# p3achyjr/p3achygo

Hardware: AMD Instinct MI355X
Metric: self-play positions/sec at 1/8 MI355X, b12c256btl3 19x19 n=32 (higher is better)
Workload: dtype f16; 1 GPU; b12c256btl3 random-init, self-play: C++ host (Gumbel MCTS n=32, default k<=5, selected k=5) -> p3hip_run over batches of 1024 leaf positions -> results back to the search; one step = one round = one engine batch of each of the 8 game groups = 8192 positions; batch_per_gpu=1024, concurrent_games_per_gpu=8192, game_groups_per_gpu=8, lanes_per_group=1, ladder_node_budget=0, parallelism=games sharded x1, no collective

## Files before the change

p3achygo_amd/csrc/conv_any.hip:

```cpp
#include "conv_any.h"

#include <hip/hip_runtime.h>

#include <atomic>
#include <cstdlib>

#include "conv_core.h"

namespace p3 {

namespace {

struct InitAnyArgs { InitArgs a; int C; };
struct Conv1x1AnyArgs { Conv1x1Args a; int cin, cout; };
struct LConvAnyArgs { LConvArgs a; int nip, ncp; };
struct BDenseAnyArgs { BDenseArgs a; int C; };

struct FeatOff {
  static constexpr int color = 4, komi = 8, board = 12, last = 376, atari = 416, two = 777,
                       three = 1138, ladder = 1499, size = 1860;
};

}

// ... 23 lines not shown
        return (_Float16)((signed char)f[off + loc] == color ? 1.0f : 0.0f);
      };
      auto opp = [&](int off) {
        return (_Float16)((signed char)f[off + loc] == -color ? 1.0f : 0.0f);
      };
      lo[0] = our(FeatOff::board); lo[1] = opp(FeatOff::board);
      lo[7] = our(FeatOff::atari); hi[0] = opp(FeatOff::atari);
      hi[1] = our(FeatOff::two); hi[2] = opp(FeatOff::two);
      hi[3] = our(FeatOff::three); hi[4] = opp(FeatOff::three);
      hi[5] = our(FeatOff::ladder); hi[6] = opp(FeatOff::ladder);
      const int y = (loc * 3450) >> 16, xx = loc - y * kBL;
#pragma unroll
      for (int m = 0; m < 5; ++m) {
        const int* lm = (const int*)(f + FeatOff::last + m * 8);
        if (lm[0] == y && lm[1] == xx) lo[2 + m] = (_Float16)1.0f;
      }
      const int s = G::PADTOP + y * G::S + xx;
      *(h8*)(smem + s * G::SLOTB) = lo;
      *(h8*)(smem + s * G::SLOTB + 16) = hi;
    }
    float gsv[8];
    gsv[0] = color == 1 ? 1.0f : 0.0f;
    gsv[1] = color == 1 ? 0.0f : 1.0f;
#pragma unroll
    for (int m = 0; m < 5; ++m) {
      const int* lm = (const int*)(f + FeatOff::last + m * 8);
      gsv[2 + m] = (lm[0] == 19 && lm[1] == 0) ? 1.0f : 0.0f;
    }
    gsv[7] = (color == 1 ? -1.0f : 1.0f) * (*(const float*)(f + FeatOff::komi)) / 15.0f;

    static_assert(kConvAnyMaxC <= kWG, "one thread per channel");
    float* bias_lds = (float*)(smem + kRingOff + ring_bytes(CP));
    const int tc = launder((int)threadIdx.x);
    if (tc < C) {
      float b = a.game_b[tc];
#pragma unroll
      for (int k = 0; k < 8; ++k) b += a.game_w[k * C + tc] * gsv[k];
      bias_lds[tc] = b;
    }

#pragma unroll 1
    for (int cp = 0; cp < C / CP; ++cp) {
      f32x16 acc[2][T::NT];
      acc_zero<G, CP>(acc);
      conv_segment<G, CP, 5, 28>(ring, smem, acc);
#pragma unroll
      for (int mt = 0; mt < 2; ++mt)
#pragma unroll
        for (int g4 = 0; g4 < 4; ++g4) {
          const int c = cp * CP + acc_chan<G, CP>(mt, g4);
          const f32x4 bias = *(const f32x4*)(bias_lds + c);
#pragma unroll
          for (int j = 0; j < T::NT; ++j) {
            const int t = lg + j * T::LG;
            if (t >= G::NT_TOTAL) continue;
            const int r = t * 32 + lr;
            int loc;
            if (!row_valid<G::S>(r, loc)) continue;
            h4 o;
#pragma unroll
            for (int i = 0; i < 4; ++i) o[i] = (_Float16)(acc[mt][j][g4 * 4 + i] + bias[i]);
            *(h4*)(a.x + ((size_t)pos * (C / 8) + (c >> 3)) * (kNLoc * 8) + loc * 8 + h * 4) = o;
          }
        }
    }
    lds_barrier();
  }
  ring_drain();
}

template <int CB, int CP, bool PRE, int EPI>
__global__ void __launch_bounds__(kWG, 2) k_conv1x1_any(Conv1x1AnyArgs aa) {
// ... 395 lines not shown
```

p3achygo_amd/csrc/conv_core.h:

```cpp
#pragma once
#include <hip/hip_runtime.h>
#include <stdint.h>

namespace p3 {

typedef _Float16 h8 __attribute__((ext_vector_type(8)));
typedef _Float16 h4 __attribute__((ext_vector_type(4)));
typedef _Float16 h2 __attribute__((ext_vector_type(2)));
typedef float f32x16 __attribute__((ext_vector_type(16)));
typedef float f32x4 __attribute__((ext_vector_type(4)));

constexpr int kWG = 512;
constexpr int kNLoc = 361;
constexpr int kBL = 19;
constexpr int kKMS = 4;
constexpr int kRingSlots = 3;
constexpr int kRingDepth = 2;
#ifndef P3_RING_DEPTH4
#define P3_RING_DEPTH4 2
#endif
constexpr int kRingDepth4 = P3_RING_DEPTH4;
constexpr int ring_slot_bytes(int cout_pass, int kms = kKMS) { return kms * cout_pass * 32; }
constexpr int ring_bytes(int cout_pass, int kms = kKMS, int depth = kRingDepth) { return (depth + 1) * ring_slot_bytes(cout_pass, kms); }

// ... 201 lines not shown

template <class G>
__device__ __forceinline__ int tile_slot0(int t) {
  int p = t / G::NT_POS;
  int tt = t - p * G::NT_POS;
  return p * G::PSLOTS + G::PADTOP + tt * 32;
}

template <int OFF>
__device__ __forceinline__ h8 lds_read128(uint32_t addr) {
  h8 r;
  asm volatile("ds_read_b128 %0, %1 offset:%2" : "=v"(r) : "v"(addr), "i"(OFF));
  return r;
}
template <int N>
__device__ __forceinline__ void wait_lgkm() {
  asm volatile("s_waitcnt lgkmcnt(%0)" ::"n"(N));
  __builtin_amdgcn_sched_barrier(0);
}

__device__ __forceinline__ void wait_lgkm_n(int n) {
  switch (n) {
    case 0: wait_lgkm<0>(); break;
    case 1: wait_lgkm<1>(); break;
    case 2: wait_lgkm<2>(); break;
    case 3: wait_lgkm<3>(); break;
    case 4: wait_lgkm<4>(); break;
    case 5: wait_lgkm<5>(); break;
    case 6: wait_lgkm<6>(); break;
    default: wait_lgkm<7>(); break;
  }
}

template <class G, int COUT_PASS, int KW, int NTAPS_PAD, bool SWAP = false, int NTn = 0>
__device__ __forceinline__ void conv_segment(Ring<ring_slot_bytes(COUT_PASS, G::KMS), G::NW, G::RD>& ring, char* smem,
                                             f32x16 (&acc)[2][NTn]) {
  using T = Tiling<G, COUT_PASS>;
  static_assert(NTn == T::NT, "accumulator shape");
  constexpr int NQ = G::CB / 16;
  constexpr int NK16 = NTAPS_PAD * NQ;
  constexpr int U = (NK16 <= 28) ? NK16 : 3 * NQ;
  constexpr int NOUT = NK16 / U;
  constexpr int NLD = 2 + T::NT;
  static_assert(NK16 % U == 0 && U % T::KMS == 0 && (NOUT == 1 || (U % 3 == 0 && U % NQ == 0)) &&
                NK16 >= 3, "segment shape");
  const int lane = threadIdx.x & 63;
  const int wid = __builtin_amdgcn_readfirstlane(threadIdx.x >> 6);
  const int cg = wid % T::CG, lg = wid / T::CG;
  const int lr = lane & 31, h = lane >> 5;

  int slot0[T::NT];
#pragma unroll
  for (int j = 0; j < T::NT; ++j) {
    int t = lg + j * T::LG;
    if (t >= G::NT_TOTAL) t = lg;
    slot0[j] = tile_slot0<G>(t) + lr;
  }
  const uint32_t a_off = (uint32_t)((h * COUT_PASS + cg * 64 + lr) * 16);
  uint32_t a_addr = 0;
  uint32_t b_base[T::NT];
  h8 fa[3][2], fb[3][T::NT];

  auto fetch_piece = [&](int o, int v, int pc) {
    const int vv = v % U;
    const int ob = o + v / U;
    const int q = vv % NQ;
    const int buf = v % 3;
    constexpr int KB = COUT_PASS * 32;
    const int kk = vv % T::KMS;
    if (pc == 0) {
      if (kk == 0) a_addr = ring_acquire(ring, smem) + a_off;
      if (vv % NQ == 0) {
        const int tap = ob * (U / NQ) + vv / NQ;
        int shift = 0;
        if (KW > 1) {
          const int ky = tap / KW, kx = tap - ky * KW;
          shift = (tap < KW * KW) ? (ky - KW / 2) * G::S + (kx - KW / 2) : 0;
        }
#pragma unroll
// ... 21 lines not shown
        case 6: fb[buf][j] = lds_read128<192>(b_base[j]); break;
        case 7: fb[buf][j] = lds_read128<224>(b_base[j]); break;
        case 8: fb[buf][j] = lds_read128<256>(b_base[j]); break;
        case 9: fb[buf][j] = lds_read128<288>(b_base[j]); break;
        case 10: fb[buf][j] = lds_read128<320>(b_base[j]); break;
        case 11: fb[buf][j] = lds_read128<352>(b_base[j]); break;
        case 12: fb[buf][j] = lds_read128<384>(b_base[j]); break;
        case 13: fb[buf][j] = lds_read128<416>(b_base[j]); break;
        case 14: fb[buf][j] = lds_read128<448>(b_base[j]); break;
        case 15: fb[buf][j] = lds_read128<480>(b_base[j]); break;
        case 16: fb[buf][j] = lds_read128<512>(b_base[j]); break;
        case 17: fb[buf][j] = lds_read128<544>(b_base[j]); break;
        case 18: fb[buf][j] = lds_read128<576>(b_base[j]); break;
        case 19: fb[buf][j] = lds_read128<608>(b_base[j]); break;
        case 20: fb[buf][j] = lds_read128<640>(b_base[j]); break;
        case 21: fb[buf][j] = lds_read128<672>(b_base[j]); break;
        case 22: fb[buf][j] = lds_read128<704>(b_base[j]); break;
        default: fb[buf][j] = lds_read128<736>(b_base[j]); break;
      }
    }
  };
  auto fetch = [&](int o, int v) {
#pragma unroll
    for (int pc = 0; pc < 1 + T::NT; ++pc) fetch_piece(o, v, pc);
  };

  fetch(0, 0);
  fetch(0, 1);
#pragma unroll 1
  for (int o = 0; o < NOUT; ++o) {
#pragma unroll
    for (int u = 0; u < U; ++u) {
      const bool last_body = (NOUT == 1) || (o + 1 == NOUT);
      if (u + 1 < U || !last_body) wait_lgkm<NLD>();
      else wait_lgkm<0>();
      const bool do_fetch = (u + 2 < U) || !last_body;
#pragma unroll
      for (int m = 0; m < 2 * T::NT; ++m) {
        const int mt = m / T::NT, j = m % T::NT;
        acc[mt][j] = SWAP ? __builtin_amdgcn_mfma_f32_32x32x16_f16(fb[u % 3][j], fa[u % 3][mt], acc[mt][j], 0, 0, 0)
                          : __builtin_amdgcn_mfma_f32_32x32x16_f16(fa[u % 3][mt], fb[u % 3][j], acc[mt][j], 0, 0, 0);
        if (m < 1 + T::NT) {
          __builtin_amdgcn_sched_barrier(0);
          if (do_fetch) fetch_piece(o, u + 2, m);
          __builtin_amdgcn_sched_barrier(0);
        }
      }
    }
  }
}

template <class G, int COUT_PASS, int NTn>
__device__ __forceinline__ void acc_zero(f32x16 (&acc)[2][NTn]) {
#pragma unroll
  for (int mt = 0; mt < 2; ++mt)
#pragma unroll
    for (int j = 0; j < NTn; ++j)
#pragma unroll
      for (int i = 0; i < 16; ++i) acc[mt][j][i] = 0.0f;
}

template <class G, int COUT_PASS>
__device__ __forceinline__ int cg_of() {
  const int wid = __builtin_amdgcn_readfirstlane(threadIdx.x >> 6);
  return wid % Tiling<G, COUT_PASS>::CG;
}

template <class G, int COUT_PASS>
__device__ __forceinline__ int acc_chan(int mt, int g4) {
// ... 256 lines not shown
                                               const ResRegs<G, COUT_PASS, NTn>& rr,
                                               _Float16* __restrict__ x) {
#pragma unroll
  for (int j = 0; j < NTn; ++j)
#pragma unroll
    for (int kp = 0; kp < 4; ++kp) {
      const int k0 = 2 * kp, k1 = 2 * kp + 1;
      h4 r0 = {0, 0, 0, 0}, r1 = {0, 0, 0, 0};
      if (RESIDUAL) residual_unpack<G, COUT_PASS, NTn>(rr, j, kp, r0, r1);
      h4 o0, o1;
#pragma unroll
      for (int i = 0; i < 4; ++i) {
        float v0 = acc[k0 >> 2][j][(k0 & 3) * 4 + i], v1 = acc[k1 >> 2][j][(k1 & 3) * 4 + i];
        if (RESIDUAL) { v0 += (float)r0[i]; v1 += (float)r1[i]; }
        o0[i] = (_Float16)v0;
        o1[i] = (_Float16)v1;
      }
      half_swap32(o0, o1);
      const h8 piece = {o0[0], o0[1], o0[2], o0[3], o1[0], o1[1], o1[2], o1[3]};
      if (rr.ok[j]) *(h8*)((char*)x + sgpr_offset(rr.pos_base * 2 + (size_t)kp * (2 * kNLoc * 8 * 2)) + (uint32_t)(rr.base[j] * 2u)) = piece;
    }
}

template <class G, int COUT_PASS, bool RESIDUAL, int NTn>
__device__ __forceinline__ void epilogue_to_global(f32x16 (&acc)[2][NTn],
                                                   _Float16* __restrict__ x, int C, int pos0,
                                                   int npos, int cofs) {
  ResRegs<G, COUT_PASS, NTn> rr;
  residual_addr<G, COUT_PASS, NTn>(rr, C, pos0, npos, cofs);
  if (RESIDUAL) residual_load<G, COUT_PASS, NTn>(rr, x);
  epilogue_store<G, COUT_PASS, RESIDUAL, NTn>(acc, rr, x);
}

}
```

p3achygo_amd/csrc/engine.cpp:

```cpp
#include <hip/hip_runtime.h>
#include <chrono>

#include <algorithm>
#include <atomic>
#include <cmath>
#include <cstdio>
#include <cstdlib>
#include <cstring>
#include <functional>
#include <map>
#include <memory>
#include <unordered_set>
#include <string>
#include <vector>

#include "../../include/p3hip.h"
#include "kernels.h"
#include "block_i8.h"
#include "conv_any.h"
#include "lconv_i8.h"
#include "slot_state.h"
#include "symmetry.h"
#include "transformer.h"

// ... 462 lines not shown
                   (C == 384 || p3::heads_fusable(C, wf.V));
  const bool arch_ok = (fused && bottleneck_ok) || layerwise || tfm ||
                       (i8f && fused_shape);
  if (!arch_ok || wf.H != 32 || !v_ok) {
    e->err = "unsupported architecture for the HIP engine (need a conv trunk (" P3HIP_CONV_SET "), or a transformer "
             "trunk (" P3HIP_TRANSFORMER_SET "); H=32, V in {32,48,64,80} (transformer: V in {32,48,64}, and 80 at "
             "d > 256))";
    return false;
  }
  if (any && e->int8) {
    e->err = std::string(e->i8f ? "INT8_FUSED" : "INT8") + " is not available for this conv trunk: P3HIP_FLAG_INT8 "
             "serves C = 384 / C_b = 192 btl or nbt blocks and C = 192 classic blocks, P3HIP_FLAG_INT8_FUSED serves "
             "C = 256 / C_b = 128 btl blocks with 1, 2 or 3 inner layers; the other widths run in fp16 only";
    return false;
  }
  e->conv_any = any || (e->conv_any_env && lw_shape && !e->int8);
  e->tfm = tfm;
  if (tfm) {
    e->tfm_heads = Cb;
    e->tfm_D = wf.model_C / Cb;
  }
  if (i8f && !i8f_ok) {
    e->err = "INT8_FUSED is available only for C = 256 / C_b = 128 trunks of btl blocks with 1, 2 or 3 inner layers "
             "(b12c256btl3 and its kin, broadcast blocks at any interval), and not together with P3HIP_FLAG_INT8; nbt and "
             "C = 128 trunks, the layer-wise trunks (P3HIP_FLAG_INT8 serves those) and the transformer are not served";
    return false;
  }
  if (e->int8 && !layerwise) {
    e->err = "INT8 is available only for layer-wise trunks (C = 384 / C_b = 192 btl or nbt blocks, C = 192 classic "
             "blocks); this trunk runs fused block kernels or the transformer";
    return false;
  }
  const int CB = layerwise ? p3::conv_any_slice(C) : (tfm ? 128 : Cb);
  const int CPI = layerwise ? p3::conv_any_init_pass(C) : 128;
  {
    std::vector<_Float16> s;
    const Tensor& w = wf.get("init_conv.w", (size_t)25 * 15 * C);
    for (int cp = 0; cp < C / CPI; ++cp)
      pack_segment(s, w.data, 25, 28, 15, C, 0, 16, cp * CPI, CPI);
    e->init_stream_off = add_stream(ar, s, e->init_nms, CPI);
    e->game_w_off = ar.add(wf.get("init_game.w", (size_t)8 * C).data, 8 * C * 4);
    e->game_b_off = ar.add(wf.get("init_game.b", (size_t)C).data, C * 4);
  }
  {
    static const bool want_blockw = getenv("P3HIP_BLOCKW") != nullptr && atoi(getenv("P3HIP_BLOCKW")) != 0;
    e->blockw = want_blockw && !i8f && C == 256 && Cb == 128 && wf.btype == 0 && wf.inner >= 1 && wf.inner <= 3;
    if (e->blockw) e->bcast_fuse = false;
  }
  bool have_xa = false;
  std::vector<std::pair<size_t, std::vector<_Float16>>> run_streams;
  std::vector<_Float16> head_stream, tail_stream;
  int head_of = -1, tail_of = -1;
  std::vector<std::function<void()>> layout;
  auto flush_run = [&]() {
    if (!run_streams.empty()) {
      auto rs_all = std::make_shared<std::vector<std::pair<size_t, std::vector<_Float16>>>>(std::move(run_streams));
      auto hs = std::make_shared<std::vector<_Float16>>(std::move(head_stream));
      auto ts = std::make_shared<std::vector<_Float16>>(std::move(tail_stream));
      const int h_of = head_of, t_of = tail_of;
      layout.push_back([&ar, e, rs_all, hs, ts, h_of, t_of, Cb]() {
        int nms_unused = 0;
        if (h_of >= 0) {
          add_stream(ar, *hs, nms_unused, Cb);
          BlockPlan& b = e->blocks[rs_all->front().first];
          b.head_of = h_of;
          b.head_bytes = hs->size() * 2;
          e->blocks[h_of].last_fused = true;
// ... 477 lines not shown
  a.prm = e->d_arena + run.prm_off;
  a.npos = npos;
  a.nblk = run.nblk;
  a.nwg = npos < e->n_cu ? npos : e->n_cu;
  a.stamps = e->d_bw_stamps;
  size_t size = sizeof a;
  void* cfg[] = {HIP_LAUNCH_PARAM_BUFFER_POINTER, &a, HIP_LAUNCH_PARAM_BUFFER_SIZE, &size, HIP_LAUNCH_PARAM_END};
  return e->check(hipModuleLaunchKernel(e->bw_fn, a.nwg, 1, 1, 256, 1, 1, 0, e->stream, nullptr, cfg), "launch k_blockw");
}

template <class Launch>
bool timed_launch(p3hip_engine* e, int* timed, Launch&& launch) {
  const bool on = timed && 2 * *timed + 1 < (int)e->blk_ev.size();
  if (on) hipEventRecord(e->blk_ev[2 * *timed], e->stream);
  if (!launch()) return false;
  if (on) hipEventRecord(e->blk_ev[2 * (*timed)++ + 1], e->stream);
  return true;
}

bool enqueue_forward(p3hip_engine* e, const Pass& p) {
  const WeightFile& wf = e->wf;
  const int C = wf.C, npos = p.npos;
  hipStream_t s = e->stream;
  const bool any = e->conv_any;
  auto conv1x1 = [&](int which, const p3::Conv1x1Args& a) {
    return any ? p3::launch_conv1x1_any(C, which, a, e->n_cu, s) : p3::launch_conv1x1(C, which, a, e->n_cu, s);
  };
  {
    p3::InitArgs a{};
    a.feats = p.feats; a.x = e->d_x; a.npos = npos;
    a.wstream = e->d_arena + e->init_stream_off; a.nms_total = e->init_nms;
    a.game_w = e->dev<float>(e->game_w_off); a.game_b = e->dev<float>(e->game_b_off);
    if (!e->check(e->conv_any ? p3::launch_init_any(C, a, grid_for(e, npos, 1), s)
                              : p3::launch_init(C, a, grid_for(e, npos, 1), s), "launch k_init")) return false;
  }
#ifdef P3_DIAG
  e->launch_index = 0;
#endif
  const int stop_block = e->stop_block;
  e->last_npos = npos;
  for (size_t bi = 0; bi < e->blocks.size(); ++bi) {
    if (stop_block >= 0 && (int)bi >= stop_block) return true;
    const BlockPlan& bp = e->blocks[bi];
    if (bp.kind == 5) {
      const int d = wf.model_C;
      const size_t per = (size_t)e->rows * p3::kTfmLPad * d;
      _Float16 *q = e->d_qkv, *k = q + per, *v = k + per, *o = e->d_t;
      p3::TfmQkvArgs a{e->d_x, q, k, v, npos, e->dev<float>(bp.tfm.rms_in), e->d_arena + bp.tfm.wqkv,
                       e->dev<float>(e->rope_cos_off), e->dev<float>(e->rope_sin_off)};
      if (!e->check(p3::launch_tfm_qkv(d, e->tfm_D, a, s), "launch k_tfm_qkv")) return false;
      const p3::TfmAttnArgs b{q, k, v, o, npos, e->tfm_heads};
      if (!timed_launch(e, p.timed, [&] { return e->check(p3::launch_tfm_attn(e->tfm_D, b, s), "launch k_tfm_attn"); }))
        return false;
      const p3::TfmFfnArgs f{o, e->d_x, npos, e->d_arena + bp.tfm.wo, e->dev<float>(bp.tfm.rms_out),
                             e->d_arena + bp.tfm.wgu, e->d_arena + bp.tfm.wdown};
      if (!e->check(p3::launch_tfm_ffn(d, f, s), "launch k_tfm_ffn")) return false;
    } else if (bp.kind == 3) {
      p3::Conv1x1Args c0{};
      c0.in = e->d_x; c0.out16 = e->d_t; c0.npos = npos;
      c0.wstream = e->d_arena + bp.stream_off; c0.nms_total = bp.nms;
      c0.scale = e->dev<float>(bp.bn[0].scale_off); c0.shift = e->dev<float>(bp.bn[0].shift_off);
      if (!bp.first_fused && !e->check(conv1x1(0, c0), "launch conv_first")) return false;
      p3::BDenseArgs d{};
      d.t = e->d_t; d.u = e->d_u; d.npos = npos;
      d.wstream = e->d_arena + bp.stream2_off; d.nms_total = bp.nms2;
      d.bias = e->dev<float>(bp.dense_bias_off);
      d.scale = e->dev<float>(bp.bn[1].scale_off); d.shift = e->dev<float>(bp.bn[1].shift_off);
// ... 790 lines not shown
```

p3achygo_amd/csrc/kernels.h:

```cpp
#pragma once
#include <hip/hip_runtime.h>
#include <stdint.h>

namespace p3 {

constexpr int kOffMoveLogits = 0;
constexpr int kOffMoveProbs = 362;
constexpr int kOffValueProbs = 724;
constexpr int kOffScoreProbs = 726;
constexpr int kOffOptProbs = 1526;
constexpr int kOffErr2 = 1888;
constexpr int kResultFloats = 1889;
constexpr int kOffOptLogits = 1889;
constexpr int kOffOutcomeLogits = 2251;
constexpr int kOffScoreLogits = 2253;
constexpr int kOffOwnership = 3053;
constexpr int kOffGamma = 3414;
constexpr int kOutStride = 3416;

constexpr int kMaxBlockLayers = 8;

constexpr int kMaxFuse = 6;
constexpr int kMaxRuns = 4, kMaxLaunchBlocks = 12;
struct BlockParams {
// ... 79 lines not shown
  const float* shift;
};

constexpr int heads_image_floats(int H, int V) {
  return 2 * H * H + 2 * H * V + 2 * H * V + (2 * H + 1) * V + V * 14 + V + V + 4 * H + 2 * H + 2 * H + H + H + H + H + H + V + V + V + 16;
}

struct HeadsArgs {
  const float* hp;
  const _Float16* x;
  const void* conv_a;
  const float* image;
  float* out;
  float* res;
  int npos;
  int V;
  const float *gbn_scale, *gbn_shift;
  const float *gd_w, *gd_b;
  const float *moves_w;
  const float *pass_w, *pass_b;
  const float *opt_moves_w;
  const float *opt_pass_w, *opt_pass_b;
  const float *oq_embed_w, *oq_embed_b;
  const float *oq_out_w, *oq_out_b;
  const float *own_w;
  const float *gamma_pre_w, *gamma_pre_b;
  const float *gamma_out_w, *gamma_out_b;
  const float *score_pre_w, *score_pre_b;
  const float *score_out_w, *score_out_b;
};

hipError_t launch_block(int C, int kind, int L, bool wg8, const BlockArgs& a, int n_cu, hipStream_t s);
int block_macro_step_bytes(int C, bool wg8);
hipError_t launch_init(int C, const InitArgs& a, int grid, hipStream_t s);
hipError_t launch_conv1x1(int C, int which, const Conv1x1Args& a, int n_cu, hipStream_t s);
hipError_t launch_bdense(int C, const BDenseArgs& a, int grid, hipStream_t s);
hipError_t launch_lconv(int kw, int cin, int cout, const LConvArgs& a, int n_cu, hipStream_t s);
hipError_t launch_heads(const HeadsArgs& a, int grid, hipStream_t s);
bool heads_fusable(int C, int V);
hipError_t launch_headsx(int C, const HeadsArgs& a, int n_cu, hipStream_t s);

constexpr int kCacheWays = 8;
struct CacheKey { unsigned long long lo, hi, sym; };
struct CacheArgs {
  const CacheKey* keys;
  int n;
  unsigned long long* tkeys;
  unsigned* tmeta;
  float* tvals;
  unsigned mask;
  unsigned run;
  int* hit;
  int* victim;
  const int* rows;
  const int* src;
  const int* idx;
  int m;
  int out_row0;
  float* out;
  unsigned* out_sym;
  const unsigned char* feats_in;
  unsigned char* feats_out;
};
hipError_t launch_cache_probe(const CacheArgs& a, hipStream_t s);
hipError_t launch_cache_gather(const CacheArgs& a, hipStream_t s);
hipError_t launch_cache_fill(const CacheArgs& a, hipStream_t s);
hipError_t launch_cache_insert(const CacheArgs& a, hipStream_t s);
// ... 4 lines not shown
```

p3achygo_amd/csrc/kernels.hip:

```cpp
#include "kernels.h"

#include <hip/hip_runtime.h>

#include <atomic>

#include "conv_core.h"
#include "conv16.h"

namespace p3 {

constexpr int kTtStride = 784;
constexpr int kTtChannels = 128;
constexpr uint32_t kTtBytes = kTtChannels * kTtStride;

struct GeoTt {
  static constexpr int NW = 8, KMS = kKMS, RD = kRingDepth;
  static constexpr int NPOS = 1, CB = 384, NCH = 48, SLOTB = kTtStride, PAD = 0, S = 1, NROWS = 128,
                       NT_POS = 4, PADTOP = 0, PSLOTS = 128, ACT_BYTES = 128 * kTtStride, NT_TOTAL = 4;
};

template <int C>
__device__ __forceinline__ void bdense_passes(Ring<16384>& ring, char* smem, const float* p_bias, const float* p_scale,
                                              const float* p_shift, _Float16* __restrict__ u, int pos, int half, int nch) {
  constexpr int CH = kTtChannels;
// ... 317 lines not shown
        residual_addr16<G, CB, NT>(xin, C, pos0, a.npos, 0);
        residual_load16<NT>(xin, a.x);
        stash16<NT>(A1, xin);
      }
      ring_note_inflight(ring, 12);
      acc16_zero<NT>(acc);
      P3_STAMP(7, 7);
      conv_segment16<G, CB, 1, 1>(ring, smem, acc);
      P3_STAMP(7, 8);
      activate_stashed16<G, CB, NT>(A1, a.tail_scale[run], a.tail_shift[run], 0);
      lds_barrier();
      epilogue_write16<G, CB, NT>(smem, A1, 0);
      P3_STAMP(7, 10);
      conv_segment16<G, CB, 1, 1>(ring, smem, acc);
      P3_STAMP(7, 11);
      lds_barrier();
      residual_addr16<G, CB, NT>(tr, C, pos0, a.npos, CB);
      epilogue_store16_mish<NT>(acc, tr, a.tout);
      P3_STAMP(7, 12);
    }
    blk0 += nblk;
    }
    P3_SPAN(2 + npos_done < 7 ? 2 + npos_done : 6);
  }
  ring_drain();
  P3_SPAN(7);
}

struct FeatOff {
  static constexpr int color = 4, komi = 8, board = 12, last = 376, atari = 416, two = 777,
                       three = 1138, ladder = 1499, size = 1860;
};

template <int C, int CP = 128>
__global__ void __launch_bounds__(kWG, 2) k_init(InitArgs a) {
  using G = Geo<1, 16, 5>;
  static_assert(C % CP == 0, "output passes");
  using T = Tiling<G, CP>;
  extern __shared__ __attribute__((aligned(16))) char smem[];
  constexpr uint32_t kRingOff = G::ACT_BYTES;
  act_zero<G>(smem);
  Ring<T::RS> ring;
  ring_init(ring, smem, a.wstream, a.nms_total, kRingOff);
  lds_barrier();
  const int lane = threadIdx.x & 63;
  const int wid = __builtin_amdgcn_readfirstlane(threadIdx.x >> 6);
  const int lg = wid / T::CG;
  const int lr = lane & 31, h = lane >> 5;

  for (int pos = blockIdx.x; pos < a.npos; pos += gridDim.x) {
    const unsigned char* f = (const unsigned char*)a.feats + (size_t)pos * FeatOff::size;
    const int color = (signed char)f[FeatOff::color];
    for (int loc = threadIdx.x; loc < kNLoc; loc += kWG) {
      h8 lo = {0, 0, 0, 0, 0, 0, 0, 0}, hi = {0, 0, 0, 0, 0, 0, 0, 0};
      auto our = [&](int off) {
        return (_Float16)((signed char)f[off + loc] == color ? 1.0f : 0.0f);
      };
      auto opp = [&](int off) {
        return (_Float16)((signed char)f[off + loc] == -color ? 1.0f : 0.0f);
      };
      lo[0] = our(FeatOff::board); lo[1] = opp(FeatOff::board);
      lo[7] = our(FeatOff::atari); hi[0] = opp(FeatOff::atari);
      hi[1] = our(FeatOff::two); hi[2] = opp(FeatOff::two);
      hi[3] = our(FeatOff::three); hi[4] = opp(FeatOff::three);
      hi[5] = our(FeatOff::ladder); hi[6] = opp(FeatOff::ladder);
      const int y = (loc * 3450) >> 16, xx = loc - y * kBL;
#pragma unroll
      for (int m = 0; m < 5; ++m) {
        const int* lm = (const int*)(f + FeatOff::last + m * 8);
        if (lm[0] == y && lm[1] == xx) lo[2 + m] = (_Float16)1.0f;
      }
      const int s = G::PADTOP + y * G::S + xx;
      *(h8*)(smem + s * G::SLOTB) = lo;
      *(h8*)(smem + s * G::SLOTB + 16) = hi;
    }
    float gsv[8];
    gsv[0] = color == 1 ? 1.0f : 0.0f;
    gsv[1] = color == 1 ? 0.0f : 1.0f;
#pragma unroll
    for (int m = 0; m < 5; ++m) {
      const int* lm = (const int*)(f + FeatOff::last + m * 8);
      gsv[2 + m] = (lm[0] == 19 && lm[1] == 0) ? 1.0f : 0.0f;
    }
    gsv[7] = (color == 1 ? -1.0f : 1.0f) * (*(const float*)(f + FeatOff::komi)) / 15.0f;

    float* bias_lds = (float*)(smem + kRingOff + ring_bytes(CP));
    if (threadIdx.x < C) {
      float b = a.game_b[threadIdx.x];
#pragma unroll
      for (int k = 0; k < 8; ++k) b += a.game_w[k * C + threadIdx.x] * gsv[k];
      bias_lds[threadIdx.x] = b;
    }

#pragma unroll 1
    for (int cp = 0; cp < C / CP; ++cp) {
      f32x16 acc[2][T::NT];
      acc_zero<G, CP>(acc);
      conv_segment<G, CP, 5, 28>(ring, smem, acc);
#pragma unroll
      for (int mt = 0; mt < 2; ++mt)
#pragma unroll
        for (int g4 = 0; g4 < 4; ++g4) {
          const int c = cp * CP + acc_chan<G, CP>(mt, g4);
          const f32x4 bias = *(const f32x4*)(bias_lds + c);
#pragma unroll
          for (int j = 0; j < T::NT; ++j) {
            const int t = lg + j * T::LG;
            if (t >= G::NT_TOTAL) continue;
            const int r = t * 32 + lr;
            int loc;
            if (!row_valid<G::S>(r, loc)) continue;
            h4 o;
#pragma unroll
            for (int i = 0; i < 4; ++i) o[i] = (_Float16)(acc[mt][j][g4 * 4 + i] + bias[i]);
            *(h4*)(a.x + ((size_t)pos * (C / 8) + (c >> 3)) * (kNLoc * 8) + loc * 8 + h * 4) = o;
          }
        }
    }
    lds_barrier();
  }
  ring_drain();
}

template <int CIN, int COUT, bool PRE, int EPI>
__global__ void __launch_bounds__(kWG, 2) k_conv1x1(Conv1x1Args a) {
  constexpr int CB = CIN >= 256 ? 128 : 64;
  constexpr int NPOS = 128 / CB;
  constexpr int CP = (COUT >= 128 && CB == 128) ? 128 : 64;
  using G = Geo<NPOS, CB, 1>;
  using T = Tiling<G, CP>;
  constexpr int NCP = (COUT + CP - 1) / CP;
  extern __shared__ __attribute__((aligned(16))) char smem[];
  constexpr uint32_t kRingOff = G::ACT_BYTES;
  act_zero<G>(smem);
  const int cp = (blockIdx.x >> 3) % NCP;
  const int pg0 = (blockIdx.x / (8 * NCP)) * 8 + (blockIdx.x & 7);
  const int pg_stride = gridDim.x / NCP;
  Ring<T::RS> ring;
  ring_init(ring, smem, (const char*)a.wstream + (size_t)cp * (a.nms_total / NCP) * T::RS, a.nms_total / NCP, kRingOff);
  lds_barrier();
  const int lane = threadIdx.x & 63;
  const int wid = __builtin_amdgcn_readfirstlane(threadIdx.x >> 6);
  const int lg = wid / T::CG;
  const int lr = lane & 31;

  constexpr int NIP = CIN / CB;
  XRegs<G> xr;
  stage_load<G>(xr, a.in, CIN, pg0 * NPOS, a.npos, 0);
  int pending_stores = 0;
  for (int pos0 = pg0 * NPOS; pos0 < a.npos; pos0 += pg_stride * NPOS) {
// ... 676 lines not shown
#pragma unroll
        for (int i = 0; i < 4; ++i) {
          const int c = 16 * u + 4 * q + i;
          gb[u][i] = sc[L::gbias + c];
          mw[u][i] = hl[L::moves_w + c * 2];
          omw[u][i] = hl[L::opt_moves_w + c];
        }
#pragma unroll
      for (int k = 0; k < TPW; ++k) {
        const int tile = wid + 4 * k;
        float pi = 0.0f, po = 0.0f;
#pragma unroll
        for (int u = 0; u < 2; ++u)
#pragma unroll
          for (int i = 0; i < 4; ++i) {
            const float pm = mish_f(P[k][u][i] + gb[u][i]);
            pi += pm * mw[u][i];
            po += pm * omw[u][i];
          }
        pi += __shfl_xor(pi, 16);
        pi += __shfl_xor(pi, 32);
        po += __shfl_xor(po, 16);
        po += __shfl_xor(po, 32);
        const int loc = tile * 16 + n;
        if (q == 0 && tile < NTILE && loc < kNLoc) {
          sc[L::pi + loc] = pi;
          sc[L::opt + loc] = po;
        }
      }
    }
    __syncthreads();
    {
      const float gam = sc[L::misc + 2];
#pragma unroll
      for (int pr = 0; pr < 2; ++pr) {
        const int s0 = t + 512 * pr, s1 = s0 + 256;
        const f32x2 sv = {0.05f * (float)(s0 - 400) + 0.025f, 0.05f * (float)(s1 - 400) + 0.025f};
        f32x2 acc = {score_out_b, score_out_b};
        const int z = launder(0);
#pragma unroll 8
        for (int k = 0; k < V; ++k) {
          const float b = sc[L::base + z + k], w = hl[L::score_pre_w + (2 * H) * V + z + k], o = hl[L::score_out_w + z + k];
          acc = __builtin_elementwise_fma(mish_f2(__builtin_elementwise_fma(sv, f32x2{w, w}, f32x2{b, b})), f32x2{o, o}, acc);
        }
        sc[L::logits + s0] = gam * acc[0];
        if (s1 < 800) sc[L::logits + s1] = gam * acc[1];
      }
    }
    __syncthreads();
    float m3[3] = {-3.0e38f, -3.0e38f, -3.0e38f};
    for (int i = t; i < 362; i += 256) {
      const float p = sc[L::pi + i], o = sc[L::opt + i];
      if (live) {
        out[kOffMoveLogits + i] = p;
        out[kOffOptLogits + i] = o;
        if (res) res[kOffMoveLogits + i] = p;
      }
      m3[0] = fmaxf(m3[0], p);
      m3[1] = fmaxf(m3[1], o);
    }
    for (int i = t; i < 800; i += 256) {
      const float l = sc[L::logits + i];
      if (live) out[kOffScoreLogits + i] = l;
      m3[2] = fmaxf(m3[2], l);
    }
#pragma unroll
    for (int r = 0; r < 3; ++r) m3[r] = wave_max(m3[r]);
    if (lane == 0) {
#pragma unroll
      for (int r = 0; r < 3; ++r) sc[L::red + r * 4 + wid] = m3[r];
    }
    __syncthreads();
#pragma unroll
    for (int r = 0; r < 3; ++r)
      m3[r] = fmaxf(fmaxf(sc[L::red + r * 4], sc[L::red + r * 4 + 1]),
                    fmaxf(sc[L::red + r * 4 + 2], sc[L::red + r * 4 + 3]));
    __syncthreads();
    float s3[3] = {0.0f, 0.0f, 0.0f};
    for (int i = t; i < 362; i += 256) {
// ... 70 lines not shown
  return hipGetLastError();
}
template <int C, int CB, int KIND, int L, int NW>
static hipError_t launch_block_t(const BlockArgs& a, int n_cu, hipStream_t s) {
  if (a.head || a.tail || a.nruns > 1) return launch_block_bc<C, CB, KIND, L, NW, true>(a, n_cu, s);
  return launch_block_bc<C, CB, KIND, L, NW, false>(a, n_cu, s);
}

int block_macro_step_bytes(int C, bool wg8) { return C == 256 ? 128 * 32 * kKMS : (wg8 ? 64 * 32 * kKMS : 64 * 32 * 2); }

hipError_t launch_block(int C, int kind, int L, bool wg8, const BlockArgs& a, int n_cu, hipStream_t s) {
  if (C == 256 && kind == 0 && L == 3) return launch_block_t<256, 128, 0, 3, 8>(a, n_cu, s);
  if (C == 256 && kind == 0 && L == 2) return launch_block_t<256, 128, 0, 2, 8>(a, n_cu, s);
  if (C == 256 && kind == 0 && L == 1) return launch_block_t<256, 128, 0, 1, 8>(a, n_cu, s);
  if (C == 256 && kind == 1) return launch_block_t<256, 128, 1, 2, 8>(a, n_cu, s);
  if (C == 128 && wg8) {
    if (kind == 0 && L == 3) return launch_block_t<128, 64, 0, 3, 8>(a, n_cu, s);
    if (kind == 0 && L == 2) return launch_block_t<128, 64, 0, 2, 8>(a, n_cu, s);
    if (kind == 0 && L == 1) return launch_block_t<128, 64, 0, 1, 8>(a, n_cu, s);
    if (kind == 1) return launch_block_t<128, 64, 1, 2, 8>(a, n_cu, s);
  }
  if (C == 128 && kind == 0 && L == 3) return launch_block_t<128, 64, 0, 3, 4>(a, n_cu, s);
  if (C == 128 && kind == 0 && L == 2) return launch_block_t<128, 64, 0, 2, 4>(a, n_cu, s);
  if (C == 128 && kind == 0 && L == 1) return launch_block_t<128, 64, 0, 1, 4>(a, n_cu, s);
  if (C == 128 && kind == 1) return launch_block_t<128, 64, 1, 2, 4>(a, n_cu, s);
  return hipErrorInvalidValue;
}

template <class K>
static hipError_t set_lds(K kernel, size_t lds) {
  return hipFuncSetAttribute((const void*)kernel, hipFuncAttributeMaxDynamicSharedMemorySize, (int)lds);
}

hipError_t launch_init(int C, const InitArgs& a, int grid, hipStream_t s) {
  using G = Geo<1, 16, 5>;
  constexpr size_t lds = G::ACT_BYTES + ring_bytes(128) + 384 * 4;
  if (C == 192) {
    constexpr size_t lds64 = G::ACT_BYTES + ring_bytes(64) + 192 * 4;
    hipLaunchKernelGGL((k_init<192, 64>), dim3(grid), dim3(kWG), lds64, s, a);
  } else if (C == 384) {
    hipLaunchKernelGGL((k_init<384>), dim3(grid), dim3(kWG), lds, s, a);
  } else if (C == 256) {
    hipLaunchKernelGGL((k_init<256>), dim3(grid), dim3(kWG), lds, s, a);
  } else if (C == 128) {
    hipLaunchKernelGGL((k_init<128>), dim3(grid), dim3(kWG), lds, s, a);
  } else {
    return hipErrorInvalidValue;
  }
  return hipGetLastError();
}

static int conv_split_grid(int npos, int npos_per_wg, int ncp, int n_cu) {
  const int unit = 8 * ncp;
  const int groups = (npos + npos_per_wg - 1) / npos_per_wg;
  int want = ((groups + 7) / 8) * unit;
  int cap = (n_cu / unit) * unit;
  if (cap < unit) cap = unit;
  return want < cap ? want : cap;
}

template <int CIN, int COUT, bool PRE, int EPI>
static hipError_t launch_conv1x1_t(const Conv1x1Args& a, int n_cu, hipStream_t s) {
  constexpr int CB = CIN >= 256 ? 128 : 64;
  using G = Geo<128 / CB, CB, 1>;
  constexpr int CP = (COUT >= 128 && CB == 128) ? 128 : 64;
  const int grid = conv_split_grid(a.npos, 128 / CB, (COUT + CP - 1) / CP, n_cu);
  constexpr size_t lds = G::ACT_BYTES + ring_bytes(CP);
  static AttrOnce once;
  if (hipError_t e = ensure_lds(once, k_conv1x1<CIN, COUT, PRE, EPI>, lds); e != hipSuccess) return e;
  hipLaunchKernelGGL((k_conv1x1<CIN, COUT, PRE, EPI>), dim3(grid), dim3(kWG), lds, s, a);
  return hipGetLastError();
}

hipError_t launch_conv1x1(int C, int which, const Conv1x1Args& a, int grid, hipStream_t s) {
  if (C == 192) {
    if (which == 0) return launch_conv1x1_t<192, 192, true, 0>(a, grid, s);
    if (which == 1) return launch_conv1x1_t<192, 192, false, 1>(a, grid, s);
    if (which == 2) return launch_conv1x1_t<192, 96, false, 2>(a, grid, s);
// ... 211 lines not shown
```

Baseline: 229,000 positions/s.

## Rework init conv kernel: prefetch feature records into LDS, skip dead taps, 64-channel passes

The init stem kernel now uses 64-channel output passes for every width and sizes its grid to two workgroups per CU. Each position's feature record is double-buffered into LDS with global_load_lds, so the next record loads while the current one is processed. The 5x5 conv segment skips the padded tap steps past the 25 live ones, and the output now goes through the shared epilogue_to_global path. Separately, the score-head loop is restructured to compute both score pairs per weight load, and the game-state bias is factored into a helper with FP contraction disabled. This adds LDS use and launch-geometry assumptions in exchange for hiding feature-load latency and cutting wasted MFMA steps in a small stage.

New measurement: 229,500 positions/s (median of 4 runs). Within noise of the previous version (+0.2%).

```diff
diff --git a/p3achygo_amd/csrc/conv_any.hip b/p3achygo_amd/csrc/conv_any.hip
--- a/p3achygo_amd/csrc/conv_any.hip
+++ b/p3achygo_amd/csrc/conv_any.hip
@@ -79,12 +79,7 @@
     static_assert(kConvAnyMaxC <= kWG, "one thread per channel");
     float* bias_lds = (float*)(smem + kRingOff + ring_bytes(CP));
     const int tc = launder((int)threadIdx.x);
-    if (tc < C) {
-      float b = a.game_b[tc];
-#pragma unroll
-      for (int k = 0; k < 8; ++k) b += a.game_w[k * C + tc] * gsv[k];
-      bias_lds[tc] = b;
-    }
+    if (tc < C) bias_lds[tc] = game_state_bias(a.game_w, a.game_b, C, tc, gsv);
 
 #pragma unroll 1
     for (int cp = 0; cp < C / CP; ++cp) {
diff --git a/p3achygo_amd/csrc/conv_core.h b/p3achygo_amd/csrc/conv_core.h
--- a/p3achygo_amd/csrc/conv_core.h
+++ b/p3achygo_amd/csrc/conv_core.h
@@ -257,7 +257,7 @@
   }
 }
 
-template <class G, int COUT_PASS, int KW, int NTAPS_PAD, bool SWAP = false, int NTn = 0>
+template <class G, int COUT_PASS, int KW, int NTAPS_PAD, bool SWAP = false, int NTn = 0, int NLIVE_ = 0>
 __device__ __forceinline__ void conv_segment(Ring<ring_slot_bytes(COUT_PASS, G::KMS), G::NW, G::RD>& ring, char* smem,
                                              f32x16 (&acc)[2][NTn]) {
   using T = Tiling<G, COUT_PASS>;
@@ -267,9 +267,12 @@
   constexpr int U = (NK16 <= 28) ? NK16 : 3 * NQ;
   constexpr int NOUT = NK16 / U;
   constexpr int NLD = 2 + T::NT;
+  constexpr int NLIVE = NLIVE_ ? NLIVE_ : NK16;
+  static_assert(NLIVE == NK16 || (NOUT == 1 && NLIVE >= 3 && NLIVE < NK16 && (NLIVE - 1) / T::KMS == (NK16 - 1) / T::KMS),
+                "dead steps: one unrolled body, all of them in the last macro-step");
   static_assert(NK16 % U == 0 && U % T::KMS == 0 && (NOUT == 1 || (U % 3 == 0 && U % NQ == 0)) &&
                 NK16 >= 3, "segment shape");
-  const int lane = threadIdx.x & 63;
+  const int lane = (KW > 1 && NOUT == 1) ? launder(threadIdx.x & 63) : (int)(threadIdx.x & 63);
   const int wid = __builtin_amdgcn_readfirstlane(threadIdx.x >> 6);
   const int cg = wid % T::CG, lg = wid / T::CG;
   const int lr = lane & 31, h = lane >> 5;
@@ -357,9 +360,10 @@
 #pragma unroll
     for (int u = 0; u < U; ++u) {
       const bool last_body = (NOUT == 1) || (o + 1 == NOUT);
-      if (u + 1 < U || !last_body) wait_lgkm<NLD>();
+      if (u >= NLIVE) continue;
+      if ((u + 1 < U && u + 1 < NLIVE) || !last_body) wait_lgkm<NLD>();
       else wait_lgkm<0>();
-      const bool do_fetch = (u + 2 < U) || !last_body;
+      const bool do_fetch = (u + 2 < U && u + 2 < NLIVE) || !last_body;
 #pragma unroll
       for (int m = 0; m < 2 * T::NT; ++m) {
         const int mt = m / T::NT, j = m % T::NT;
@@ -682,4 +686,13 @@
   epilogue_store<G, COUT_PASS, RESIDUAL, NTn>(acc, rr, x);
 }
 
-}
+__device__ __forceinline__ float game_state_bias(const float* __restrict__ game_w, const float* __restrict__ game_b,
+                                                 int C, int c, const float (&gsv)[8]) {
+#pragma clang fp contract(off)
+  float b = game_b[c];
+#pragma unroll
+  for (int k = 0; k < 8; ++k) b = b + game_w[k * C + c] * gsv[k];
+  return b;
+}
+
+}
diff --git a/p3achygo_amd/csrc/engine.cpp b/p3achygo_amd/csrc/engine.cpp
--- a/p3achygo_amd/csrc/engine.cpp
+++ b/p3achygo_amd/csrc/engine.cpp
@@ -518,7 +518,7 @@
     return false;
   }
   const int CB = layerwise ? p3::conv_any_slice(C) : (tfm ? 128 : Cb);
-  const int CPI = layerwise ? p3::conv_any_init_pass(C) : 128;
+  const int CPI = e->conv_any ? p3::conv_any_init_pass(C) : p3::kInitPass;
   {
     std::vector<_Float16> s;
     const Tensor& w = wf.get("init_conv.w", (size_t)25 * 15 * C);
@@ -1062,7 +1062,7 @@
     a.wstream = e->d_arena + e->init_stream_off; a.nms_total = e->init_nms;
     a.game_w = e->dev<float>(e->game_w_off); a.game_b = e->dev<float>(e->game_b_off);
     if (!e->check(e->conv_any ? p3::launch_init_any(C, a, grid_for(e, npos, 1), s)
-                              : p3::launch_init(C, a, grid_for(e, npos, 1), s), "launch k_init")) return false;
+                              : p3::launch_init(C, a, e->n_cu, s), "launch k_init")) return false;
   }
 #ifdef P3_DIAG
   e->launch_index = 0;
diff --git a/p3achygo_amd/csrc/kernels.h b/p3achygo_amd/csrc/kernels.h
--- a/p3achygo_amd/csrc/kernels.h
+++ b/p3achygo_amd/csrc/kernels.h
@@ -135,7 +135,8 @@
 
 hipError_t launch_block(int C, int kind, int L, bool wg8, const BlockArgs& a, int n_cu, hipStream_t s);
 int block_macro_step_bytes(int C, bool wg8);
-hipError_t launch_init(int C, const InitArgs& a, int grid, hipStream_t s);
+constexpr int kInitPass = 64;
+hipError_t launch_init(int C, const InitArgs& a, int n_cu, hipStream_t s);
 hipError_t launch_conv1x1(int C, int which, const Conv1x1Args& a, int n_cu, hipStream_t s);
 hipError_t launch_bdense(int C, const BDenseArgs& a, int grid, hipStream_t s);
 hipError_t launch_lconv(int kw, int cin, int cout, const LConvArgs& a, int n_cu, hipStream_t s);
diff --git a/p3achygo_amd/csrc/kernels.hip b/p3achygo_amd/csrc/kernels.hip
--- a/p3achygo_amd/csrc/kernels.hip
+++ b/p3achygo_amd/csrc/kernels.hip
@@ -373,27 +373,48 @@
                        three = 1138, ladder = 1499, size = 1860;
 };
 
-template <int C, int CP = 128>
-__global__ void __launch_bounds__(kWG, 2) k_init(InitArgs a) {
+struct InitLds {
   using G = Geo<1, 16, 5>;
-  static_assert(C % CP == 0, "output passes");
+  static constexpr int kRecWords = FeatOff::size / 4, kRecBuf = kWG * 4;
+  static constexpr uint32_t ring = G::ACT_BYTES, bias = ring + ring_bytes(kInitPass), rec = bias + 384 * 4,
+                            bytes = rec + 2 * kRecBuf;
+  static_assert(FeatOff::size % 4 == 0 && kRecWords <= kWG, "one dword of the record per thread");
+  static_assert(2 * bytes <= 160 * 1024, "k_init: two workgroups per CU");
+};
+
+template <int C>
+__global__ void __launch_bounds__(kWG, 4) k_init(InitArgs a) {
+  using G = InitLds::G;
+  constexpr int CP = kInitPass;
+  static_assert(C % CP == 0 && C <= 384, "output passes");
   using T = Tiling<G, CP>;
   extern __shared__ __attribute__((aligned(16))) char smem[];
-  constexpr uint32_t kRingOff = G::ACT_BYTES;
   act_zero<G>(smem);
   Ring<T::RS> ring;
-  ring_init(ring, smem, a.wstream, a.nms_total, kRingOff);
+  ring_init(ring, smem, a.wstream, a.nms_total, InitLds::ring);
+  auto rec_fetch = [&](int pos, int buf) {
+    const int t = launder((int)threadIdx.x);
+    const int w = t < InitLds::kRecWords ? t : InitLds::kRecWords - 1;
+    const int wid = __builtin_amdgcn_readfirstlane(t >> 6);
+    __builtin_amdgcn_global_load_lds(
+        (const __attribute__((address_space(1))) void*)((const char*)a.feats + (size_t)pos * FeatOff::size + w * 4),
+        (__attribute__((address_space(3))) void*)(smem + InitLds::rec + buf * InitLds::kRecBuf + wid * 256), 4, 0, 0);
+  };
+  if ((int)blockIdx.x < a.npos) rec_fetch(blockIdx.x, 0);
+  ring_drain();
   lds_barrier();
-  const int lane = threadIdx.x & 63;
-  const int wid = __builtin_amdgcn_readfirstlane(threadIdx.x >> 6);
-  const int lg = wid / T::CG;
-  const int lr = lane & 31, h = lane >> 5;
-
-  for (int pos = blockIdx.x; pos < a.npos; pos += gridDim.x) {
-    const unsigned char* f = (const unsigned char*)a.feats + (size_t)pos * FeatOff::size;
+
+  int buf = 0;
+  for (int pos = blockIdx.x; pos < a.npos; pos += gridDim.x, buf ^= 1) {
+    const int tid = launder((int)threadIdx.x);
+    const unsigned char* f = (const unsigned char*)(smem + InitLds::rec + buf * InitLds::kRecBuf);
+    rec_fetch(pos + (int)gridDim.x < a.npos ? pos + (int)gridDim.x : pos, buf ^ 1);
     const int color = (signed char)f[FeatOff::color];
-    for (int loc = threadIdx.x; loc < kNLoc; loc += kWG) {
-      h8 lo = {0, 0, 0, 0, 0, 0, 0, 0}, hi = {0, 0, 0, 0, 0, 0, 0, 0};
+    static_assert(kNLoc <= kWG, "one thread per board point");
+    if (tid < kNLoc) {
+      const int loc = tid;
+      const float z = __builtin_bit_cast(float, launder(0));
+      h8 lo = __builtin_bit_cast(h8, f32x4{z, z, z, z}), hi = lo;
       auto our = [&](int off) {
         return (_Float16)((signed char)f[off + loc] == color ? 1.0f : 0.0f);
       };
@@ -425,38 +446,27 @@
     }
     gsv[7] = (color == 1 ? -1.0f : 1.0f) * (*(const float*)(f + FeatOff::komi)) / 15.0f;
 
-    float* bias_lds = (float*)(smem + kRingOff + ring_bytes(CP));
-    if (threadIdx.x < C) {
-      float b = a.game_b[threadIdx.x];
-#pragma unroll
-      for (int k = 0; k < 8; ++k) b += a.game_w[k * C + threadIdx.x] * gsv[k];
-      bias_lds[threadIdx.x] = b;
-    }
+    float* bias_lds = (float*)(smem + InitLds::bias);
+    if (tid < C) bias_lds[tid] = game_state_bias(a.game_w, a.game_b, C, tid, gsv);
 
 #pragma unroll 1
     for (int cp = 0; cp < C / CP; ++cp) {
       f32x16 acc[2][T::NT];
       acc_zero<G, CP>(acc);
-      conv_segment<G, CP, 5, 28>(ring, smem, acc);
+      conv_segment<G, CP, 5, 28, false, T::NT, 25>(ring, smem, acc);
+      static_assert(T::CG == 1, "acc_chan below");
+      const int hc = (launder((int)threadIdx.x & 63) >> 5) * 4;
 #pragma unroll
       for (int mt = 0; mt < 2; ++mt)
 #pragma unroll
         for (int g4 = 0; g4 < 4; ++g4) {
-          const int c = cp * CP + acc_chan<G, CP>(mt, g4);
-          const f32x4 bias = *(const f32x4*)(bias_lds + c);
-#pragma unroll
-          for (int j = 0; j < T::NT; ++j) {
-            const int t = lg + j * T::LG;
-            if (t >= G::NT_TOTAL) continue;
-            const int r = t * 32 + lr;
-            int loc;
-            if (!row_valid<G::S>(r, loc)) continue;
-            h4 o;
-#pragma unroll
-            for (int i = 0; i < 4; ++i) o[i] = (_Float16)(acc[mt][j][g4 * 4 + i] + bias[i]);
-            *(h4*)(a.x + ((size_t)pos * (C / 8) + (c >> 3)) * (kNLoc * 8) + loc * 8 + h * 4) = o;
-          }
-        }
+          const f32x4 bias = *(const f32x4*)(bias_lds + cp * CP + mt * 32 + g4 * 8 + hc);
+#pragma unroll
+          for (int j = 0; j < T::NT; ++j)
+#pragma unroll
+            for (int i = 0; i < 4; ++i) acc[mt][j][g4 * 4 + i] += bias[i];
+        }
+      epilogue_to_global<G, CP, false>(acc, a.x, C, pos, a.npos, cp * CP);
     }
     lds_barrier();
   }
@@ -1199,19 +1209,26 @@
     __syncthreads();
     {
       const float gam = sc[L::misc + 2];
+      f32x2 sv[2], acc[2];
 #pragma unroll
       for (int pr = 0; pr < 2; ++pr) {
         const int s0 = t + 512 * pr, s1 = s0 + 256;
-        const f32x2 sv = {0.05f * (float)(s0 - 400) + 0.025f, 0.05f * (float)(s1 - 400) + 0.025f};
-        f32x2 acc = {score_out_b, score_out_b};
-        const int z = launder(0);
+        sv[pr] = f32x2{0.05f * (float)(s0 - 400) + 0.025f, 0.05f * (float)(s1 - 400) + 0.025f};
+        acc[pr] = f32x2{score_out_b, score_out_b};
+      }
+      const int z = launder(0);
 #pragma unroll 8
-        for (int k = 0; k < V; ++k) {
-          const float b = sc[L::base + z + k], w = hl[L::score_pre_w + (2 * H) * V + z + k], o = hl[L::score_out_w + z + k];
-          acc = __builtin_elementwise_fma(mish_f2(__builtin_elementwise_fma(sv, f32x2{w, w}, f32x2{b, b})), f32x2{o, o}, acc);
-        }
-        sc[L::logits + s0] = gam * acc[0];
-        if (s1 < 800) sc[L::logits + s1] = gam * acc[1];
+      for (int k = 0; k < V; ++k) {
+        const float b = sc[L::base + z + k], w = hl[L::score_pre_w + (2 * H) * V + z + k], o = hl[L::score_out_w + z + k];
+#pragma unroll
+        for (int pr = 0; pr < 2; ++pr)
+          acc[pr] = __builtin_elementwise_fma(mish_f2(__builtin_elementwise_fma(sv[pr], f32x2{w, w}, f32x2{b, b})), f32x2{o, o}, acc[pr]);
+      }
+#pragma unroll
+      for (int pr = 0; pr < 2; ++pr) {
+        const int s0 = t + 512 * pr, s1 = s0 + 256;
+        sc[L::logits + s0] = gam * acc[pr][0];
+        if (s1 < 800) sc[L::logits + s1] = gam * acc[pr][1];
       }
     }
     __syncthreads();
@@ -1348,18 +1365,16 @@
   return hipFuncSetAttribute((const void*)kernel, hipFuncAttributeMaxDynamicSharedMemorySize, (int)lds);
 }
 
-hipError_t launch_init(int C, const InitArgs& a, int grid, hipStream_t s) {
-  using G = Geo<1, 16, 5>;
-  constexpr size_t lds = G::ACT_BYTES + ring_bytes(128) + 384 * 4;
-  if (C == 192) {
-    constexpr size_t lds64 = G::ACT_BYTES + ring_bytes(64) + 192 * 4;
-    hipLaunchKernelGGL((k_init<192, 64>), dim3(grid), dim3(kWG), lds64, s, a);
-  } else if (C == 384) {
-    hipLaunchKernelGGL((k_init<384>), dim3(grid), dim3(kWG), lds, s, a);
+hipError_t launch_init(int C, const InitArgs& a, int n_cu, hipStream_t s) {
+  const int grid = a.npos < 2 * n_cu ? a.npos : 2 * n_cu;
+  if (C == 384) {
+    hipLaunchKernelGGL((k_init<384>), dim3(grid), dim3(kWG), InitLds::bytes, s, a);
   } else if (C == 256) {
-    hipLaunchKernelGGL((k_init<256>), dim3(grid), dim3(kWG), lds, s, a);
+    hipLaunchKernelGGL((k_init<256>), dim3(grid), dim3(kWG), InitLds::bytes, s, a);
+  } else if (C == 192) {
+    hipLaunchKernelGGL((k_init<192>), dim3(grid), dim3(kWG), InitLds::bytes, s, a);
   } else if (C == 128) {
-    hipLaunchKernelGGL((k_init<128>), dim3(grid), dim3(kWG), lds, s, a);
+    hipLaunchKernelGGL((k_init<128>), dim3(grid), dim3(kWG), InitLds::bytes, s, a);
   } else {
     return hipErrorInvalidValue;
   }
```
